# DCASE-REPO/DESED_task

Measured on AMD Instinct MI355X. Metric: 10s-clips/sec CRNN mean-teacher train @batch48, higher is better.
Workload: dtype f32 (fp32 storage and accumulation; the dense contractions of the wide layers run as split-bf16 MFMA, 3 bf16 products per fp32 product, fp32-level accuracy; everything else exact f32)

## Files before the change

desed_task_amd/csrc/sed_block0.hip:

```cpp
#include "sed_common.h"

#define B0_TR 16
#define B0_MAXF 128
#define B0_PITCH(F) ((F) + 8)

template <int BATCH>
__device__ __forceinline__ void b0_stage(float* tile, const float* __restrict__ x, const int* __restrict__ bounds, int b, int t0, int T,
                                         int F, float center) {
    if constexpr (BATCH >= 8) {
        if (sed_stage_halo_f4<B0_TR, 256, B0_MAXF>(tile, x, bounds, b, t0, T, F, B0_PITCH(F), center)) return;
    }
    const int PW = F + 2, PT = B0_PITCH(F), n = (B0_TR + 2) * PW;
    int mf0 = 0, mf1 = 0, mt0 = 0, mt1 = 0;
    if (bounds) { mf0 = bounds[4 * b]; mf1 = bounds[4 * b + 1]; mt0 = bounds[4 * b + 2]; mt1 = bounds[4 * b + 3]; }
    for (int base = threadIdx.x; base < n; base += 256 * BATCH) {
        float v[BATCH];
        bool ok[BATCH];
        int pad[BATCH];
#pragma unroll
        for (int u = 0; u < BATCH; ++u) {
            const int idx = base + 256 * u, ic = idx < n ? idx : n - 1;
            const int i = ic / PW, j = ic - i * PW;
            const int t = t0 - 1 + i, f = j - 1;
            const int tc = t < 0 ? 0 : (t >= T ? T - 1 : t), fc = f < 0 ? 0 : (f >= F ? F - 1 : f);
            v[u] = x[((size_t)b * T + tc) * F + fc];
            pad[u] = i * (PT - PW);
            ok[u] = t >= 0 && t < T && f >= 0 && f < F && !((f >= mf0 && f < mf1) || (t >= mt0 && t < mt1));
        }
        sed_sched_fence();
#pragma unroll
        for (int u = 0; u < BATCH; ++u) sed_pin(v[u]);
#pragma unroll
        for (int u = 0; u < BATCH; ++u) {
            const int idx = base + 256 * u;
            if (idx < n) tile[idx + pad[u]] = (ok[u] ? v[u] : 0.f) - center;
        }
    }
}

__global__ __launch_bounds__(256) void block0_fwd_kernel(const float* __restrict__ x, const float* __restrict__ W,
                                                         const float* __restrict__ bias, const int* __restrict__ bounds,
                                                         const float* __restrict__ stats, const float* __restrict__ Wg,
                                                         const float* __restrict__ bg, float* __restrict__ out, int B, int T, int F,
                                                         uint32_t seed, uint32_t thr24, float dscale,
                                                         const unsigned* __restrict__ seed_dev) {
    if (seed_dev) seed += *seed_dev;
    constexpr int C = 16;
    __shared__ float tile[(B0_TR + 2) * B0_PITCH(B0_MAXF)];
    const int lane = threadIdx.x & 63, i = lane & 15, g = lane >> 4, wv = threadIdx.x >> 6;
    const int b = blockIdx.y, t0 = blockIdx.x * B0_TR, PW = B0_PITCH(F);
    float wreg[4][9], breg[4], wa[4], sc[4], sh[4], bgr[4];
#pragma unroll
    for (int c = 0; c < 4; ++c) {
        breg[c] = bias ? bias[4 * g + c] : 0.f;
#pragma unroll
        for (int k = 0; k < 9; ++k) wreg[c][k] = W[(4 * g + c) * 9 + k];
        wa[c] = Wg[i * C + 4 * g + c];
        sc[c] = stats[2 * C + 4 * g + c];
        sh[c] = stats[3 * C + 4 * g + c];
        bgr[c] = bg[4 * g + c];
    }
    b0_stage<10>(tile, x, bounds, b, t0, T, F, 0.f);
    __syncthreads();
    const int To = T / 2, Fo = F / 2, tpr = Fo / 4;
    const int w = i >> 2, q = i & 3;
    for (int pr = wv; pr < B0_TR / 2; pr += 4) {
        const int to = (t0 >> 1) + pr;
        if (to >= To) break;
        const int lr = 2 * pr + (q >> 1);
        for (int tr = 0; tr < tpr; ++tr) {
            const int col = 2 * (4 * tr + w) + (q & 1);
            float in[9];
#pragma unroll
            for (int a = 0; a < 3; ++a)
#pragma unroll
                for (int bb = 0; bb < 3; ++bb) in[a * 3 + bb] = tile[(lr + a) * PW + col + bb];
            float xn[4];
#pragma unroll
            for (int c = 0; c < 4; c += 2) {
                f32x2 acc2 = {0.f, 0.f};
#pragma unroll
                for (int k = 0; k < 9; ++k) acc2 = pk_fma(f32x2{in[k], in[k]}, f32x2{wreg[c][k], wreg[c + 1][k]}, acc2);
                const float a0 = acc2.x + breg[c], a1 = acc2.y + breg[c + 1];
                xn[c] = fmaf(a0, sc[c], sh[c]);
                xn[c + 1] = fmaf(a1, sc[c + 1], sh[c + 1]);
            }
            f32x4 acc = {0.f, 0.f, 0.f, 0.f};
#pragma unroll
            for (int k = 0; k < 4; ++k) acc = mfma16(wa[k], xn[k], acc);
            const size_t pix = ((size_t)b * T + t0 + lr) * F + col;
            float v[4];
#pragma unroll
            for (int r = 0; r < 4; ++r) {
                float o = (acc[r] + bgr[r]) * sed_fast_sigmoid(xn[r]);
                const uint32_t e = (uint32_t)(pix * C + 4 * g + r);
                o = sed_keep(e, seed, thr24) ? o * dscale : 0.f;
                v[r] = 0.25f * sed_quad_sum(o);
            }
            if (q == 0)
                *(float4*)(out + (((size_t)b * To + to) * Fo + 4 * tr + w) * C + 4 * g) = make_float4(v[0], v[1], v[2], v[3]);
        }
    }
}

SED_API int sed_block0_fwd(const float* x, const float* W, const float* bias, const int* bounds, const float* stats,
                              const float* Wg, const float* bg, float* out, int B, int T, int F, unsigned seed, unsigned thr24,
                              float dscale, const unsigned* seed_dev, void* stream) {
    if (F > B0_MAXF || F < 8 || F % 8 != 0) return SED_ERR_UNSUPPORTED;
    if (B <= 0 || T < 2) return SED_OK;
    SED_LAUNCH(block0_fwd_kernel, dim3((T + B0_TR - 1) / B0_TR, B), dim3(256), 0, (hipStream_t)stream, x, W, bias, bounds, stats, Wg,
               bg, out, B, T, F, seed, thr24, dscale, seed_dev);
    return sed_check_launch();
}

#define B0_O_DBG 256
#define B0_O_DGAM 272
#define B0_O_DBET 288
#define B0_O_S1 304
#define B0_O_S2 448
#define B0_O_XH 592
#define B0_O_SX 608
#define B0_O_K 617
#define B0_O_CNT 618
#define B0_NP 624
#define B0_NSUM 617

#ifndef B0_BWD_BATCH
#define B0_BWD_BATCH 4
#endif
#define B0_TS 20
__global__ __launch_bounds__(256, 2) void block0_bwd_kernel(const float* __restrict__ x, const float* __restrict__ W,
                                                         const float* __restrict__ bias, const int* __restrict__ bounds,
                                                         const float* __restrict__ stats, const float* __restrict__ gamma,
                                                         const float* __restrict__ beta, const float* __restrict__ Wg,
                                                         const float* __restrict__ bg, const float* __restrict__ gout,
                                                         float* __restrict__ part, int B, int T, int F, int tiles_t, uint32_t seed,
                                                         uint32_t thr24, float dscale, const unsigned* __restrict__ seed_dev,
                                                         int center) {
    if (seed_dev) seed += *seed_dev;
    constexpr int C = 16;
    __shared__ float tile[(B0_TR + 2) * B0_PITCH(B0_MAXF)];
    __shared__ float red[4][B0_NP];
    __shared__ __attribute__((aligned(16))) float tbuf[4][2][16 * B0_TS];
    __shared__ float kred[4];
    const int lane = threadIdx.x & 63, i = lane & 15, g = lane >> 4, wv = threadIdx.x >> 6;
    const int PW = B0_PITCH(F), ntiles = B * tiles_t;
    const int To = T / 2, Fo = F / 2, tpr = Fo / 4;
    float k;
    {
        const int tl = blockIdx.x, b = tl / tiles_t, t0 = (tl - b * tiles_t) * B0_TR;
        float s = 0.f;
        int n = 0;
#pragma unroll
        for (int u = 0; u < B0_TR * B0_MAXF / 512; ++u) {
            const int idx = threadIdx.x + 512 * u, ic = idx < B0_TR * F ? idx : 0;
            const int r = ic / F, f = ic - r * F, t = t0 + r;
            const float xv = x[((size_t)b * T + (t < T ? t : T - 1)) * F + f];
            if (idx < B0_TR * F && t < T) { s += xv; ++n; }
        }
        float nf = (float)n;
        s = wave_sum(s); nf = wave_sum(nf);
        if (lane == 0) { kred[wv] = s; red[wv][0] = nf; }
        __syncthreads();
        const float tot = sed_sadd(sed_sadd(kred[0], kred[1]), sed_sadd(kred[2], kred[3]));
        const float cnt = sed_sadd(sed_sadd(red[0][0], red[1][0]), sed_sadd(red[2][0], red[3][0]));
        k = (center && cnt > 0.f) ? tot / cnt : 0.f;
        __syncthreads();
    }
    float wreg[4][9], breg[4], wa1[4], wb2[4], mu[4], istd[4], gam4[4], bet4[4], bgr[4];
#pragma unroll
    for (int c = 0; c < 4; ++c) {
        const int ch = 4 * g + c;
        float ws = 0.f;
#pragma unroll
        for (int kk = 0; kk < 9; ++kk) { wreg[c][kk] = W[ch * 9 + kk]; ws += wreg[c][kk]; }
        breg[c] = (bias ? bias[ch] : 0.f) + k * ws;
        wa1[c] = Wg[i * C + ch];
        wb2[c] = Wg[ch * C + i];
        mu[c] = stats[ch]; istd[c] = stats[C + ch];
        gam4[c] = gamma[ch]; bet4[c] = beta[ch];
        bgr[c] = bg[ch];
    }
#pragma unroll
    for (int c = 0; c < 4; ++c) {
#pragma unroll
        for (int kk = 0; kk < 9; ++kk) sed_pin(wreg[c][kk]);
        sed_pin(breg[c]); sed_pin(wa1[c]); sed_pin(wb2[c]); sed_pin(mu[c]); sed_pin(istd[c]); sed_pin(gam4[c]); sed_pin(bet4[c]); sed_pin(bgr[c]);
    }
    f32x4 P = {0.f, 0.f, 0.f, 0.f};
    float a_dgam[4], a_dbet[4], a_dbg[4], a_xh[4], a_sx[9], a_cnt = 0.f;
    f32x2 S12[4][9];
#pragma unroll
    for (int c = 0; c < 4; ++c) {
        a_dgam[c] = 0.f; a_dbet[c] = 0.f; a_dbg[c] = 0.f; a_xh[c] = 0.f;
#pragma unroll
        for (int kk = 0; kk < 9; ++kk) S12[c][kk] = f32x2{0.f, 0.f};
    }
#pragma unroll
    for (int kk = 0; kk < 9; ++kk) a_sx[kk] = 0.f;
    const int w = i >> 2, q = i & 3;
    float* t1 = tbuf[wv][0];
    float* t2 = tbuf[wv][1];
    for (int tl = blockIdx.x; tl < ntiles; tl += gridDim.x) {
        const int b = tl / tiles_t, t0 = (tl - b * tiles_t) * B0_TR;
        __syncthreads();
        b0_stage<B0_BWD_BATCH>(tile, x, bounds, b, t0, T, F, k);
        __syncthreads();
        for (int pr = wv; pr < B0_TR / 2; pr += 4) {
            const int to = (t0 >> 1) + pr;
            const bool tail = (to == To) && (T & 1);
            if (to >= To && !tail) break;
            const int lr = 2 * pr + (q >> 1);
            const float vm = (tail && (q >> 1)) ? 0.f : 1.f;
            const float gsc = tail ? 0.f : 0.25f * dscale;
            const float* grow = gout + (((size_t)b * To + (tail ? To - 1 : to)) * Fo + w) * C + 4 * g;
            float4 go_n = *(const float4*)grow;
            for (int tr = 0; tr < tpr; ++tr) {
                const float4 go = go_n;
                go_n = *(const float4*)(grow + (size_t)(4 * C) * (tr + 1 < tpr ? tr + 1 : tr));
                const int col = 2 * (4 * tr + w) + (q & 1);
                float in[9];
#pragma unroll
                for (int a = 0; a < 3; ++a)
#pragma unroll
                    for (int bb = 0; bb < 3; ++bb) in[a * 3 + bb] = tile[(lr + a) * PW + col + bb];
                float xh[4], xn[4];
#pragma unroll
                for (int c = 0; c < 4; c += 2) {
                    f32x2 acc2 = {0.f, 0.f};
#pragma unroll
                    for (int kk = 0; kk < 9; ++kk) acc2 = pk_fma(f32x2{in[kk], in[kk]}, f32x2{wreg[c][kk], wreg[c + 1][kk]}, acc2);
                    const float a0 = acc2.x + breg[c], a1 = acc2.y + breg[c + 1];
                    xh[c] = (a0 - mu[c]) * istd[c] * vm;
                    xh[c + 1] = (a1 - mu[c + 1]) * istd[c + 1] * vm;
                    xn[c] = fmaf(xh[c], gam4[c], bet4[c]);
                    xn[c + 1] = fmaf(xh[c + 1], gam4[c + 1], bet4[c + 1]);
                }
                f32x4 acc1 = {0.f, 0.f, 0.f, 0.f};
#pragma unroll
                for (int kk = 0; kk < 4; ++kk) acc1 = mfma16(wa1[kk], xn[kk], acc1);
                const float gv[4] = {go.x, go.y, go.z, go.w};
                const size_t pix = ((size_t)b * T + t0 + lr) * F + col;
                float dlin[4], e[4];
#pragma unroll
                for (int r = 0; r < 4; ++r) {
                    const float lin = acc1[r] + bgr[r];
                    const float sg = sed_fast_sigmoid(xn[r]);
                    const uint32_t ei = (uint32_t)(pix * C + 4 * g + r);
                    const float gr = sed_keep(ei, seed, thr24) ? gv[r] * gsc : 0.f;
                    dlin[r] = gr * sg;
                    e[r] = gr * lin * sg * (1.0f - sg);
                }
                sed_wave_sync();
                *(float4*)(t1 + i * B0_TS + 4 * g) = make_float4(dlin[0], dlin[1], dlin[2], dlin[3]);
                *(float4*)(t2 + i * B0_TS + 4 * g) = make_float4(xn[0], xn[1], xn[2], xn[3]);
                f32x4 acc2 = {0.f, 0.f, 0.f, 0.f};
#pragma unroll
                for (int kk = 0; kk < 4; ++kk) acc2 = mfma16(wb2[kk], dlin[kk], acc2);
#pragma unroll
                for (int r = 0; r < 4; ++r) {
                    const float dxn = acc2[r] + e[r];
                    a_dgam[r] = fmaf(dxn, xh[r], a_dgam[r]);
                    a_dbet[r] += dxn;
                    a_dbg[r] += dlin[r];
                    a_xh[r] += xh[r];
                    const float dzr = dxn * gam4[r];
#pragma unroll
                    for (int kk = 0; kk < 9; ++kk) {
                        S12[r][kk] = pk_fma(f32x2{in[kk], in[kk]}, f32x2{dzr, xh[r]}, S12[r][kk]);
                    }
                }
#pragma unroll
                for (int kk = 0; kk < 9; ++kk) a_sx[kk] = fmaf(in[kk], vm, a_sx[kk]);
                a_cnt += vm;
                sed_wave_sync();
                float dT[4], xT[4];
#pragma unroll
                for (int kk = 0; kk < 4; ++kk) { dT[kk] = t1[(4 * g + kk) * B0_TS + i]; xT[kk] = t2[(4 * g + kk) * B0_TS + i]; }
#pragma unroll
                for (int kk = 0; kk < 4; ++kk) P = mfma16(dT[kk], xT[kk], P);
            }
        }
    }
#pragma unroll
    for (int r = 0; r < 4; ++r) red[wv][(4 * g + r) * C + i] = P[r];
#pragma unroll
    for (int m = 1; m <= 8; m <<= 1) {
#pragma unroll
        for (int c = 0; c < 4; ++c) {
            a_dgam[c] += __shfl_xor(a_dgam[c], m); a_dbet[c] += __shfl_xor(a_dbet[c], m);
            a_dbg[c] += __shfl_xor(a_dbg[c], m); a_xh[c] += __shfl_xor(a_xh[c], m);
#pragma unroll
            for (int kk = 0; kk < 9; ++kk) { S12[c][kk].x += __shfl_xor(S12[c][kk].x, m); S12[c][kk].y += __shfl_xor(S12[c][kk].y, m); }
        }
#pragma unroll
        for (int kk = 0; kk < 9; ++kk) a_sx[kk] += __shfl_xor(a_sx[kk], m);
        a_cnt += __shfl_xor(a_cnt, m);
    }
    if (i == 0) {
#pragma unroll
        for (int c = 0; c < 4; ++c) {
            const int ch = 4 * g + c;
            red[wv][B0_O_DBG + ch] = a_dbg[c]; red[wv][B0_O_DGAM + ch] = a_dgam[c]; red[wv][B0_O_DBET + ch] = a_dbet[c];
            red[wv][B0_O_XH + ch] = a_xh[c];
#pragma unroll
            for (int kk = 0; kk < 9; ++kk) { red[wv][B0_O_S1 + ch * 9 + kk] = S12[c][kk].x; red[wv][B0_O_S2 + ch * 9 + kk] = S12[c][kk].y; }
        }
        if (g == 0) {
#pragma unroll
            for (int kk = 0; kk < 9; ++kk) red[wv][B0_O_SX + kk] = a_sx[kk];
            red[wv][B0_O_CNT] = a_cnt; red[wv][B0_O_K] = 0.f;
        }
    }
    __syncthreads();
    for (int idx = threadIdx.x; idx < B0_NP; idx += 256) {
        float v = (red[0][idx] + red[1][idx]) + (red[2][idx] + red[3][idx]);
        if (idx == B0_O_K) v = k;
        if (idx > B0_O_CNT) v = 0.f;
        part[(size_t)blockIdx.x * B0_NP + idx] = v;
    }
}

__global__ __launch_bounds__(1024) void block0_bwd_reduce_kernel(const float* __restrict__ part, int nparts,
                                                                 const float* __restrict__ gamma, double* __restrict__ sums) {
    __shared__ double red[32][33];
    const int tid = threadIdx.x, col = tid & 31, grp = tid >> 5, o = blockIdx.x * 32 + col;
    double acc = 0.0;
    if (o < B0_NP) {
        int o2 = -1;
        float scale = 1.0f;
        if (o >= B0_O_S1 && o < B0_O_S2) { const int c = (o - B0_O_S1) / 9; o2 = B0_O_DBET + c; scale = gamma[c]; }
        else if (o >= B0_O_S2 && o < B0_O_XH) { const int c = (o - B0_O_S2) / 9; o2 = B0_O_XH + c; }
        else if (o >= B0_O_SX && o < B0_O_K) o2 = B0_O_CNT;
        if (o2 >= 0) {
#pragma unroll 4
            for (int p = grp; p < nparts; p += 32) {
                const float* rec = part + (size_t)p * B0_NP;
                acc += (double)rec[o] + (double)rec[B0_O_K] * (double)scale * (double)rec[o2];
            }
        } else {
#pragma unroll 4
            for (int p = grp; p < nparts; p += 32) acc += (double)part[(size_t)p * B0_NP + o];
        }
    }
    red[grp][col] = acc;
    __syncthreads();
    if (grp == 0 && o < B0_NP) {
#pragma unroll
        for (int gq = 1; gq < 32; ++gq) acc += red[gq][col];
        sums[o] = acc;
    }
}

__global__ __launch_bounds__(256) void block0_bwd_final_kernel(const double* __restrict__ sums, const float* __restrict__ stats,
                                                               const float* __restrict__ gamma, float* __restrict__ dW,
                                                               float* __restrict__ dbias, float* __restrict__ dgamma,
                                                               float* __restrict__ dbeta, float* __restrict__ dWg,
                                                               float* __restrict__ dbg, double count) {
    constexpr int C = 16;
    const int tid = threadIdx.x;
    dWg[tid] = (float)sums[tid];
    if (tid < C) {
        dbg[tid] = (float)sums[B0_O_DBG + tid];
        dgamma[tid] = (float)sums[B0_O_DGAM + tid];
        dbeta[tid] = (float)sums[B0_O_DBET + tid];
        if (dbias) dbias[tid] = 0.f;
    }
    if (tid < C * 9) {
        const int c = tid / 9, tap = tid - 9 * c;
        const double g = (double)gamma[c], is = (double)stats[C + c];
        const double m1 = g * sums[B0_O_DBET + c] / count, m2 = g * sums[B0_O_DGAM + c] / count;
        dW[tid] = (float)(is * (sums[B0_O_S1 + tid] - m1 * sums[B0_O_SX + tap] - m2 * sums[B0_O_S2 + tid]));
    }
}

static inline int block0_bwd_grid(int B, int T) {
    const int ntiles = B * ((T + B0_TR - 1) / B0_TR);
    const int forced = sed_tuning[SED_TUNE_GLU_GRID_CAP];
    const int cap = forced > 0 ? forced : 512;
    return ntiles < cap ? ntiles : cap;
}
SED_API long long sed_block0_bwd_scratch_floats(int B, int T, int F) {
    (void)F;
    return (long long)block0_bwd_grid(B, T) * B0_NP + 2 * B0_NP + 2;
}

SED_API int sed_block0_bwd(const float* x, const float* W, const float* bias, const int* bounds, const float* stats,
                              const float* gamma, const float* beta, const float* Wg, const float* bg, const float* gout,
                              float* dW, float* dbias, float* dgamma, float* dbeta, float* dWg, float* dbg, float* scratch, int B,
                              int T, int F, unsigned seed, unsigned thr24, float dscale, const unsigned* seed_dev, void* stream) {
    if (F > B0_MAXF || F < 8 || F % 8 != 0) return SED_ERR_UNSUPPORTED;
    hipStream_t s = (hipStream_t)stream;
    const int grid = block0_bwd_grid(B, T);
    if (grid < 1 || T < 2) {
        sed_zero4(s, dWg, 256, dW, 144, dgamma, 16, dbeta, 16);
        sed_zero4(s, dbg, 16, dbias, dbias ? 16 : 0, nullptr, 0, nullptr, 0);
        return sed_check_launch();
    }
    if (!scratch) return SED_ERR_ARG;
    const int tiles_t = (T + B0_TR - 1) / B0_TR;
    float* part = scratch;
    size_t off = (size_t)grid * B0_NP;
    off += off & 1;
    double* sums = (double*)(scratch + off);
    SED_LAUNCH(block0_bwd_kernel, dim3(grid), dim3(256), 0, s, x, W, bias, bounds, stats, gamma, beta, Wg, bg, gout, part, B, T, F,
               tiles_t, seed, thr24, dscale, seed_dev, sed_tuning[SED_TUNE_B0_NOCENTER] ? 0 : 1);
    SED_LAUNCH(block0_bwd_reduce_kernel, dim3((B0_NP + 31) / 32), dim3(1024), 0, s, (const float*)part, grid, gamma, sums);
    SED_LAUNCH(block0_bwd_final_kernel, dim3(1), dim3(256), 0, s, (const double*)sums, stats, gamma, dW, dbias, dgamma, dbeta, dWg, dbg,
               (double)B * (double)T * (double)F);
    return sed_check_launch();
}
```

Baseline: 16780.

## Move block0 backward conv and weight-gradient accumulations onto MFMA, raise occupancy

The backward kernel for the first conv+BN+GLU block now computes the 3x3 conv forward recompute with three MFMA ops instead of per-thread packed FMAs. It also accumulates the dW statistics (S1/S2, sums of xh and dxn) through MFMA outer products over transposed LDS buffers, replacing 72 pinned accumulator pairs per thread. The gamma scale moves from the reduce kernel into the final kernel. The tile pitch becomes a compile-time constant, the reduction buffer aliases the transpose buffers, and launch bounds rise to 4 blocks per CU with the grid sized from the queried occupancy. This cuts VGPR pressure and FMA work in exchange for extra LDS traffic and wave syncs per step, and the reformulated accumulation may round differently.

Result: no change. 16770 (median of 2 runs) (-0.1%).

```diff
diff --git a/desed_task_amd/csrc/sed_block0.hip b/desed_task_amd/csrc/sed_block0.hip
--- a/desed_task_amd/csrc/sed_block0.hip
+++ b/desed_task_amd/csrc/sed_block0.hip
@@ -6,11 +6,11 @@
 
 template <int BATCH>
 __device__ __forceinline__ void b0_stage(float* tile, const float* __restrict__ x, const int* __restrict__ bounds, int b, int t0, int T,
-                                         int F, float center) {
+                                         int F, int PT, float center) {
     if constexpr (BATCH >= 8) {
-        if (sed_stage_halo_f4<B0_TR, 256, B0_MAXF>(tile, x, bounds, b, t0, T, F, B0_PITCH(F), center)) return;
-    }
-    const int PW = F + 2, PT = B0_PITCH(F), n = (B0_TR + 2) * PW;
+        if (sed_stage_halo_f4<B0_TR, 256, B0_MAXF>(tile, x, bounds, b, t0, T, F, PT, center)) return;
+    }
+    const int PW = F + 2, n = (B0_TR + 2) * PW;
     int mf0 = 0, mf1 = 0, mt0 = 0, mt1 = 0;
     if (bounds) { mf0 = bounds[4 * b]; mf1 = bounds[4 * b + 1]; mt0 = bounds[4 * b + 2]; mt1 = bounds[4 * b + 3]; }
     for (int base = threadIdx.x; base < n; base += 256 * BATCH) {
@@ -60,7 +60,7 @@
         sh[c] = stats[3 * C + 4 * g + c];
         bgr[c] = bg[4 * g + c];
     }
-    b0_stage<10>(tile, x, bounds, b, t0, T, F, 0.f);
+    b0_stage<10>(tile, x, bounds, b, t0, T, F, PW, 0.f);
     __syncthreads();
     const int To = T / 2, Fo = F / 2, tpr = Fo / 4;
     const int w = i >> 2, q = i & 3;
@@ -128,8 +128,16 @@
 #ifndef B0_BWD_BATCH
 #define B0_BWD_BATCH 4
 #endif
+__device__ __forceinline__ float b0_xor(float v, int lt, int m) {
+#ifdef SED_EMU
+    (void)lt;
+    return __shfl_xor(v, m);
+#else
+    return __builtin_bit_cast(float, __builtin_amdgcn_ds_bpermute(((lt & 63) ^ m) << 2, __builtin_bit_cast(int, v)));
+#endif
+}
 #define B0_TS 20
-__global__ __launch_bounds__(256, 2) void block0_bwd_kernel(const float* __restrict__ x, const float* __restrict__ W,
+__global__ __launch_bounds__(256, 4) void block0_bwd_kernel(const float* __restrict__ x, const float* __restrict__ W,
                                                          const float* __restrict__ bias, const int* __restrict__ bounds,
                                                          const float* __restrict__ stats, const float* __restrict__ gamma,
                                                          const float* __restrict__ beta, const float* __restrict__ Wg,
@@ -140,11 +148,13 @@
     if (seed_dev) seed += *seed_dev;
     constexpr int C = 16;
     __shared__ float tile[(B0_TR + 2) * B0_PITCH(B0_MAXF)];
-    __shared__ float red[4][B0_NP];
-    __shared__ __attribute__((aligned(16))) float tbuf[4][2][16 * B0_TS];
+    __shared__ __attribute__((aligned(16))) float tbuf[4][4][16 * B0_TS];
     __shared__ float kred[4];
+    static_assert(4 * B0_NP <= 4 * 4 * 16 * B0_TS, "partial records must fit the transposition buffers");
+    float (*red)[B0_NP] = reinterpret_cast<float (*)[B0_NP]>(&tbuf[0][0][0]);
     const int lane = threadIdx.x & 63, i = lane & 15, g = lane >> 4, wv = threadIdx.x >> 6;
-    const int PW = B0_PITCH(F), ntiles = B * tiles_t;
+    constexpr int PW = B0_PITCH(B0_MAXF);
+    const int ntiles = B * tiles_t;
     const int To = T / 2, Fo = F / 2, tpr = Fo / 4;
     float k;
     {
@@ -167,44 +177,45 @@
         k = (center && cnt > 0.f) ? tot / cnt : 0.f;
         __syncthreads();
     }
-    float wreg[4][9], breg[4], wa1[4], wb2[4], mu[4], istd[4], gam4[4], bet4[4], bgr[4];
+    float wc[3], bm[4], wa1[4], wb2[4], istd[4], gam4[4], bet4[4], bgr[4];
+    wc[0] = W[i * 9 + g];
+    wc[1] = W[i * 9 + 4 + g];
+    wc[2] = g == 0 ? W[i * 9 + 8] : 0.f;
 #pragma unroll
     for (int c = 0; c < 4; ++c) {
         const int ch = 4 * g + c;
         float ws = 0.f;
 #pragma unroll
-        for (int kk = 0; kk < 9; ++kk) { wreg[c][kk] = W[ch * 9 + kk]; ws += wreg[c][kk]; }
-        breg[c] = (bias ? bias[ch] : 0.f) + k * ws;
+        for (int kk = 0; kk < 9; ++kk) ws += W[ch * 9 + kk];
+        bm[c] = (bias ? bias[ch] : 0.f) + k * ws - stats[ch];
         wa1[c] = Wg[i * C + ch];
         wb2[c] = Wg[ch * C + i];
-        mu[c] = stats[ch]; istd[c] = stats[C + ch];
+        istd[c] = stats[C + ch];
         gam4[c] = gamma[ch]; bet4[c] = beta[ch];
         bgr[c] = bg[ch];
     }
 #pragma unroll
+    for (int s = 0; s < 3; ++s) sed_pin(wc[s]);
+#pragma unroll
     for (int c = 0; c < 4; ++c) {
-#pragma unroll
-        for (int kk = 0; kk < 9; ++kk) sed_pin(wreg[c][kk]);
-        sed_pin(breg[c]); sed_pin(wa1[c]); sed_pin(wb2[c]); sed_pin(mu[c]); sed_pin(istd[c]); sed_pin(gam4[c]); sed_pin(bet4[c]); sed_pin(bgr[c]);
-    }
-    f32x4 P = {0.f, 0.f, 0.f, 0.f};
-    float a_dgam[4], a_dbet[4], a_dbg[4], a_xh[4], a_sx[9], a_cnt = 0.f;
-    f32x2 S12[4][9];
-#pragma unroll
-    for (int c = 0; c < 4; ++c) {
-        a_dgam[c] = 0.f; a_dbet[c] = 0.f; a_dbg[c] = 0.f; a_xh[c] = 0.f;
-#pragma unroll
-        for (int kk = 0; kk < 9; ++kk) S12[c][kk] = f32x2{0.f, 0.f};
-    }
-#pragma unroll
-    for (int kk = 0; kk < 9; ++kk) a_sx[kk] = 0.f;
+        sed_pin(bm[c]); sed_pin(wa1[c]); sed_pin(wb2[c]); sed_pin(istd[c]); sed_pin(gam4[c]); sed_pin(bet4[c]); sed_pin(bgr[c]);
+    }
+    const int oc0 = (g / 3) * PW + g % 3, oc1 = ((4 + g) / 3) * PW + (4 + g) % 3, oc2 = 2 * PW + 2;
+    const int os = i < 9 ? (i / 3) * PW + i % 3 : 0;
+    const float bone = i == 9 ? 1.f : 0.f;
+    f32x4 P = {0.f, 0.f, 0.f, 0.f}, S1 = {0.f, 0.f, 0.f, 0.f}, S2 = {0.f, 0.f, 0.f, 0.f};
+    float a_dgam[4], a_dbg[4], a_sx = 0.f;
+#pragma unroll
+    for (int c = 0; c < 4; ++c) { a_dgam[c] = 0.f; a_dbg[c] = 0.f; }
     const int w = i >> 2, q = i & 3;
     float* t1 = tbuf[wv][0];
     float* t2 = tbuf[wv][1];
+    float* t3 = tbuf[wv][2];
+    float* t4 = tbuf[wv][3];
     for (int tl = blockIdx.x; tl < ntiles; tl += gridDim.x) {
         const int b = tl / tiles_t, t0 = (tl - b * tiles_t) * B0_TR;
         __syncthreads();
-        b0_stage<B0_BWD_BATCH>(tile, x, bounds, b, t0, T, F, k);
+        b0_stage<B0_BWD_BATCH>(tile, x, bounds, b, t0, T, F, PW, k);
         __syncthreads();
         for (int pr = wv; pr < B0_TR / 2; pr += 4) {
             const int to = (t0 >> 1) + pr;
@@ -219,22 +230,23 @@
                 const float4 go = go_n;
                 go_n = *(const float4*)(grow + (size_t)(4 * C) * (tr + 1 < tpr ? tr + 1 : tr));
                 const int col = 2 * (4 * tr + w) + (q & 1);
-                float in[9];
-#pragma unroll
-                for (int a = 0; a < 3; ++a)
-#pragma unroll
-                    for (int bb = 0; bb < 3; ++bb) in[a * 3 + bb] = tile[(lr + a) * PW + col + bb];
+                const float* tp = tile + lr * PW + col;
+                const float* sp = tile + 2 * pr * PW + 8 * tr + 2 * g + os;
+                float xb[4];
+#pragma unroll
+                for (int kk = 0; kk < 4; ++kk) {
+                    const float v = sp[(kk >> 1) * PW + (kk & 1)];
+                    xb[kk] = (tail && (kk >> 1)) ? 0.f : (i < 9 ? v : bone);
+                }
+                f32x4 y = {0.f, 0.f, 0.f, 0.f};
+                y = mfma16(wc[0], tp[oc0], y);
+                y = mfma16(wc[1], tp[oc1], y);
+                y = mfma16(wc[2], tp[oc2], y);
                 float xh[4], xn[4];
 #pragma unroll
-                for (int c = 0; c < 4; c += 2) {
-                    f32x2 acc2 = {0.f, 0.f};
-#pragma unroll
-                    for (int kk = 0; kk < 9; ++kk) acc2 = pk_fma(f32x2{in[kk], in[kk]}, f32x2{wreg[c][kk], wreg[c + 1][kk]}, acc2);
-                    const float a0 = acc2.x + breg[c], a1 = acc2.y + breg[c + 1];
-                    xh[c] = (a0 - mu[c]) * istd[c] * vm;
-                    xh[c + 1] = (a1 - mu[c + 1]) * istd[c + 1] * vm;
+                for (int c = 0; c < 4; ++c) {
+                    xh[c] = (y[c] + bm[c]) * istd[c] * vm;
                     xn[c] = fmaf(xh[c], gam4[c], bet4[c]);
-                    xn[c + 1] = fmaf(xh[c + 1], gam4[c + 1], bet4[c + 1]);
                 }
                 f32x4 acc1 = {0.f, 0.f, 0.f, 0.f};
 #pragma unroll
@@ -251,66 +263,61 @@
                     dlin[r] = gr * sg;
                     e[r] = gr * lin * sg * (1.0f - sg);
                 }
+                f32x4 acc2 = {0.f, 0.f, 0.f, 0.f};
+#pragma unroll
+                for (int kk = 0; kk < 4; ++kk) acc2 = mfma16(wb2[kk], dlin[kk], acc2);
+                float dxn[4];
+#pragma unroll
+                for (int r = 0; r < 4; ++r) {
+                    dxn[r] = acc2[r] + e[r];
+                    a_dgam[r] = fmaf(dxn[r], xh[r], a_dgam[r]);
+                    a_dbg[r] += dlin[r];
+                }
+                a_sx += (xb[0] + xb[1]) + (xb[2] + xb[3]);
                 sed_wave_sync();
                 *(float4*)(t1 + i * B0_TS + 4 * g) = make_float4(dlin[0], dlin[1], dlin[2], dlin[3]);
                 *(float4*)(t2 + i * B0_TS + 4 * g) = make_float4(xn[0], xn[1], xn[2], xn[3]);
-                f32x4 acc2 = {0.f, 0.f, 0.f, 0.f};
-#pragma unroll
-                for (int kk = 0; kk < 4; ++kk) acc2 = mfma16(wb2[kk], dlin[kk], acc2);
-#pragma unroll
-                for (int r = 0; r < 4; ++r) {
-                    const float dxn = acc2[r] + e[r];
-                    a_dgam[r] = fmaf(dxn, xh[r], a_dgam[r]);
-                    a_dbet[r] += dxn;
-                    a_dbg[r] += dlin[r];
-                    a_xh[r] += xh[r];
-                    const float dzr = dxn * gam4[r];
-#pragma unroll
-                    for (int kk = 0; kk < 9; ++kk) {
-                        S12[r][kk] = pk_fma(f32x2{in[kk], in[kk]}, f32x2{dzr, xh[r]}, S12[r][kk]);
-                    }
+                *(float4*)(t3 + i * B0_TS + 4 * g) = make_float4(dxn[0], dxn[1], dxn[2], dxn[3]);
+                *(float4*)(t4 + i * B0_TS + 4 * g) = make_float4(xh[0], xh[1], xh[2], xh[3]);
+                sed_wave_sync();
+                float dT[4], xT[4], nT[4], hT[4];
+#pragma unroll
+                for (int kk = 0; kk < 4; ++kk) {
+                    const int o = (4 * g + kk) * B0_TS + i;
+                    dT[kk] = t1[o]; xT[kk] = t2[o]; nT[kk] = t3[o]; hT[kk] = t4[o];
                 }
 #pragma unroll
-                for (int kk = 0; kk < 9; ++kk) a_sx[kk] = fmaf(in[kk], vm, a_sx[kk]);
-                a_cnt += vm;
-                sed_wave_sync();
-                float dT[4], xT[4];
-#pragma unroll
-                for (int kk = 0; kk < 4; ++kk) { dT[kk] = t1[(4 * g + kk) * B0_TS + i]; xT[kk] = t2[(4 * g + kk) * B0_TS + i]; }
-#pragma unroll
                 for (int kk = 0; kk < 4; ++kk) P = mfma16(dT[kk], xT[kk], P);
+#pragma unroll
+                for (int kk = 0; kk < 4; ++kk) S1 = mfma16(nT[kk], xb[kk], S1);
+#pragma unroll
+                for (int kk = 0; kk < 4; ++kk) S2 = mfma16(hT[kk], xb[kk], S2);
             }
         }
     }
-#pragma unroll
-    for (int r = 0; r < 4; ++r) red[wv][(4 * g + r) * C + i] = P[r];
-#pragma unroll
-    for (int m = 1; m <= 8; m <<= 1) {
-#pragma unroll
-        for (int c = 0; c < 4; ++c) {
-            a_dgam[c] += __shfl_xor(a_dgam[c], m); a_dbet[c] += __shfl_xor(a_dbet[c], m);
-            a_dbg[c] += __shfl_xor(a_dbg[c], m); a_xh[c] += __shfl_xor(a_xh[c], m);
-#pragma unroll
-            for (int kk = 0; kk < 9; ++kk) { S12[c][kk].x += __shfl_xor(S12[c][kk].x, m); S12[c][kk].y += __shfl_xor(S12[c][kk].y, m); }
-        }
-#pragma unroll
-        for (int kk = 0; kk < 9; ++kk) a_sx[kk] += __shfl_xor(a_sx[kk], m);
-        a_cnt += __shfl_xor(a_cnt, m);
-    }
-    if (i == 0) {
-#pragma unroll
-        for (int c = 0; c < 4; ++c) {
-            const int ch = 4 * g + c;
-            red[wv][B0_O_DBG + ch] = a_dbg[c]; red[wv][B0_O_DGAM + ch] = a_dgam[c]; red[wv][B0_O_DBET + ch] = a_dbet[c];
-            red[wv][B0_O_XH + ch] = a_xh[c];
-#pragma unroll
-            for (int kk = 0; kk < 9; ++kk) { red[wv][B0_O_S1 + ch * 9 + kk] = S12[c][kk].x; red[wv][B0_O_S2 + ch * 9 + kk] = S12[c][kk].y; }
-        }
-        if (g == 0) {
-#pragma unroll
-            for (int kk = 0; kk < 9; ++kk) red[wv][B0_O_SX + kk] = a_sx[kk];
-            red[wv][B0_O_CNT] = a_cnt; red[wv][B0_O_K] = 0.f;
-        }
+    __syncthreads();
+    int lt = threadIdx.x;
+    sed_opaque(lt);
+    const int ri = lt & 15, rg = (lt & 63) >> 4;
+#pragma unroll
+    for (int r = 0; r < 4; ++r) {
+        const int ch = 4 * rg + r;
+        red[wv][ch * C + ri] = P[r];
+        if (ri < 9) { red[wv][B0_O_S1 + ch * 9 + ri] = S1[r]; red[wv][B0_O_S2 + ch * 9 + ri] = S2[r]; }
+        else if (ri == 9) { red[wv][B0_O_DBET + ch] = S1[r]; red[wv][B0_O_XH + ch] = S2[r]; }
+    }
+#pragma unroll
+    for (int c = 0; c < 4; ++c) { a_dgam[c] = sed_row16_sum(a_dgam[c]); a_dbg[c] = sed_row16_sum(a_dbg[c]); }
+    a_sx += b0_xor(a_sx, lt, 16);
+    a_sx += b0_xor(a_sx, lt, 32);
+    if (ri == 0) {
+#pragma unroll
+        for (int c = 0; c < 4; ++c) { red[wv][B0_O_DBG + 4 * rg + c] = a_dbg[c]; red[wv][B0_O_DGAM + 4 * rg + c] = a_dgam[c]; }
+    }
+    if (rg == 0) {
+        if (ri < 9) red[wv][B0_O_SX + ri] = a_sx;
+        else if (ri == 9) red[wv][B0_O_CNT] = a_sx;
+        else if (ri == 10) red[wv][B0_O_K] = 0.f;
     }
     __syncthreads();
     for (int idx = threadIdx.x; idx < B0_NP; idx += 256) {
@@ -321,22 +328,20 @@
     }
 }
 
-__global__ __launch_bounds__(1024) void block0_bwd_reduce_kernel(const float* __restrict__ part, int nparts,
-                                                                 const float* __restrict__ gamma, double* __restrict__ sums) {
+__global__ __launch_bounds__(1024) void block0_bwd_reduce_kernel(const float* __restrict__ part, int nparts, double* __restrict__ sums) {
     __shared__ double red[32][33];
     const int tid = threadIdx.x, col = tid & 31, grp = tid >> 5, o = blockIdx.x * 32 + col;
     double acc = 0.0;
     if (o < B0_NP) {
         int o2 = -1;
-        float scale = 1.0f;
-        if (o >= B0_O_S1 && o < B0_O_S2) { const int c = (o - B0_O_S1) / 9; o2 = B0_O_DBET + c; scale = gamma[c]; }
+        if (o >= B0_O_S1 && o < B0_O_S2) o2 = B0_O_DBET + (o - B0_O_S1) / 9;
         else if (o >= B0_O_S2 && o < B0_O_XH) { const int c = (o - B0_O_S2) / 9; o2 = B0_O_XH + c; }
         else if (o >= B0_O_SX && o < B0_O_K) o2 = B0_O_CNT;
         if (o2 >= 0) {
 #pragma unroll 4
             for (int p = grp; p < nparts; p += 32) {
                 const float* rec = part + (size_t)p * B0_NP;
-                acc += (double)rec[o] + (double)rec[B0_O_K] * (double)scale * (double)rec[o2];
+                acc += (double)rec[o] + (double)rec[B0_O_K] * (double)rec[o2];
             }
         } else {
 #pragma unroll 4
@@ -370,14 +375,31 @@
         const int c = tid / 9, tap = tid - 9 * c;
         const double g = (double)gamma[c], is = (double)stats[C + c];
         const double m1 = g * sums[B0_O_DBET + c] / count, m2 = g * sums[B0_O_DGAM + c] / count;
-        dW[tid] = (float)(is * (sums[B0_O_S1 + tid] - m1 * sums[B0_O_SX + tap] - m2 * sums[B0_O_S2 + tid]));
-    }
-}
-
+        dW[tid] = (float)(is * (g * sums[B0_O_S1 + tid] - m1 * sums[B0_O_SX + tap] - m2 * sums[B0_O_S2 + tid]));
+    }
+}
+
+static int block0_bwd_slots() {
+#ifdef SED_EMU
+    return 1024;
+#else
+    static int slots = 0;
+    if (slots == 0) {
+        int per_cu = 0, dev = 0;
+        hipDeviceProp_t prop;
+        if (hipGetDevice(&dev) != hipSuccess || hipGetDeviceProperties(&prop, dev) != hipSuccess ||
+            hipOccupancyMaxActiveBlocksPerMultiprocessor(&per_cu, (const void*)block0_bwd_kernel, 256, 0) != hipSuccess || per_cu < 1)
+            slots = 1024;
+        else
+            slots = per_cu * prop.multiProcessorCount;
+    }
+    return slots;
+#endif
+}
 static inline int block0_bwd_grid(int B, int T) {
     const int ntiles = B * ((T + B0_TR - 1) / B0_TR);
     const int forced = sed_tuning[SED_TUNE_GLU_GRID_CAP];
-    const int cap = forced > 0 ? forced : 512;
+    const int cap = forced > 0 ? forced : block0_bwd_slots();
     return ntiles < cap ? ntiles : cap;
 }
 SED_API long long sed_block0_bwd_scratch_floats(int B, int T, int F) {
@@ -405,7 +427,7 @@
     double* sums = (double*)(scratch + off);
     SED_LAUNCH(block0_bwd_kernel, dim3(grid), dim3(256), 0, s, x, W, bias, bounds, stats, gamma, beta, Wg, bg, gout, part, B, T, F,
                tiles_t, seed, thr24, dscale, seed_dev, sed_tuning[SED_TUNE_B0_NOCENTER] ? 0 : 1);
-    SED_LAUNCH(block0_bwd_reduce_kernel, dim3((B0_NP + 31) / 32), dim3(1024), 0, s, (const float*)part, grid, gamma, sums);
+    SED_LAUNCH(block0_bwd_reduce_kernel, dim3((B0_NP + 31) / 32), dim3(1024), 0, s, (const float*)part, grid, sums);
     SED_LAUNCH(block0_bwd_final_kernel, dim3(1), dim3(256), 0, s, (const double*)sums, stats, gamma, dW, dbias, dgamma, dbeta, dWg, dbg,
                (double)B * (double)T * (double)F);
     return sed_check_launch();
```
